# byuccl/coast

Hardware: NVIDIA B200
Metric: protected-kernel throughput (MB/s voted output), sha256 TMR (higher is better)
Workload: dtype u32

## Files before the change

### coast_b200/csrc/coast_rt.c

```c
#define _GNU_SOURCE
#include "../../include/coast_rt.h"
#include "xmr_args.h"

#include <cuda.h>
#include <ctype.h>
#include <dlfcn.h>
#include <sched.h>
#include <stdarg.h>
#include <stdio.h>
#include <stdlib.h>
#include <string.h>
#include <sys/syscall.h>
#include <unistd.h>

extern const unsigned char coast_kernels_cubin[];

__attribute__((weak)) uint32_t TMR_ERROR_CNT = 0;
__attribute__((weak)) uint64_t __SYNC_COUNT = 0;
__attribute__((weak)) void FAULT_DETECTED_DWC(void) {
    fprintf(stderr, "coast_rt: DWC mismatch detected -> FAULT_DETECTED_DWC -> abort()\n");
    abort();
}

#define DRV_FUNCS(X)                                                                                         \
// ... 469 lines not shown
    char name[64];
    snprintf(name, sizeof name, "xmr_mm_u32_%s_nc%u_inj%d", atmem ? "tct" : "tc", nc, inj);
    CUfunction fn; int occ = 1;
    int rc = get_fn(name, smem, &fn, &occ); if (rc) return rc;
    CUtensorMap ma, mb;
    {
        cuuint64_t gdim[3] = { d->K, d->M, 4 };
        cuuint64_t gstr[2] = { (cuuint64_t)d->K, (cuuint64_t)d->M * d->K };
        cuuint32_t box[3] = { 128, 128, 4 };
        cuuint32_t estr[3] = { 1, 1, 1 };
        DRV(p_cuTensorMapEncodeTiled(&ma, CU_TENSOR_MAP_DATA_TYPE_UINT8, 3, (void*)pa, gdim, gstr, box, estr,
                                     CU_TENSOR_MAP_INTERLEAVE_NONE, CU_TENSOR_MAP_SWIZZLE_128B,
                                     CU_TENSOR_MAP_L2_PROMOTION_L2_256B, CU_TENSOR_MAP_FLOAT_OOB_FILL_NONE));
    }
    {
        cuuint64_t gdim[3] = { d->K, d->N, 4 };
        cuuint64_t gstr[2] = { (cuuint64_t)d->K, (cuuint64_t)d->N * d->K };
        cuuint32_t box[3] = { 128, bn, 4 };
        cuuint32_t estr[3] = { 1, 1, 1 };
        DRV(p_cuTensorMapEncodeTiled(&mb, CU_TENSOR_MAP_DATA_TYPE_UINT8, 3, (void*)pb, gdim, gstr, box, estr,
                                     CU_TENSOR_MAP_INTERLEAVE_NONE, CU_TENSOR_MAP_SWIZZLE_128B,
                                     CU_TENSOR_MAP_L2_PROMOTION_L2_256B, CU_TENSOR_MAP_FLOAT_OOB_FILL_NONE));
    }
    unsigned tiles = (d->M / 128u) * (d->N / bn);
    unsigned grid = tiles < (unsigned)G.sm_count ? tiles : (unsigned)G.sm_count;
    void* params[3] = { a, &ma, &mb };
    if (d->flags & COAST_F_VERBOSE) fprintf(stderr, "coast_rt: %s grid=%u smem=%u tiles=%u\n", name, grid, smem, tiles);
    DRV(p_cuLaunchKernel(fn, grid, 1, 1, 256, 1, 1, smem, stream, params, NULL));
    return COAST_OK;
}
static int launch_mm_tc(const coast_launch_desc* d, xmr_args* a, int inj, CUstream stream, int atmem) {
    const size_t a_bytes = (size_t)d->M * d->K * 4u, b_bytes = (size_t)d->K * d->N * 4u;
    CUdeviceptr planes = 0;
    DRV(p_cuMemAllocFromPoolAsync(&planes, a_bytes + b_bytes, G.pool, stream));
    int rc = launch_mm_tc_planes(d, a, inj, stream, atmem, planes, planes + a_bytes);
    p_cuMemFreeAsync(planes, stream);
    return rc;
}

static int launch_impl(const coast_launch_desc* d, void* stream) {
    int rc = ensure_ctx(); if (rc) return rc;
    if (!d) return fail(COAST_ERR_BAD_ARG, "null descriptor");
    if (d->kernel >= COAST_K_COUNT_) return fail(COAST_ERR_BAD_ARG, "unknown kernel id %u", d->kernel);
    if (d->num_clones < 1 || d->num_clones > 3) return fail(COAST_ERR_BAD_ARG, "num_clones must be 1, 2 (DWC) or 3 (TMR)");
    if (d->n_units == 0) return COAST_OK;
    if (!d->d_in || !d->d_out) return fail(COAST_ERR_BAD_ARG, "null device buffer");
    const uint32_t nc = d->num_clones;
    const uint32_t upw = 32u / nc;
    const int inj = d->plan && d->plan->mode != COAST_PLAN_NONE;

    xmr_args a; memset(&a, 0, sizeof a);
    a.in = d->d_in; a.out = d->d_out; a.aux = d->d_aux;
    a.n_units = d->n_units; a.unit_base = d->unit_base;
    a.counters = (unsigned long long*)(G.peer_counters ? G.peer_counters : G.counters);
    a.status = (unsigned char*)d->d_status;
    a.unit_bytes = d->unit_bytes; a.flags = d->flags; a.mode = d->mode;
    a.M = d->M; a.N = d->N; a.K = d->K;
    memcpy(a.key, d->key, 16);
    if (inj) {
        a.plan_mode = d->plan->mode; a.seed_lo = d->plan->seed_lo; a.seed_hi = d->plan->seed_hi;
        a.threshold = d->plan->threshold; a.plan_table = (const unsigned int*)d->plan->d_table;
        if (a.plan_mode == COAST_PLAN_TABLE && !a.plan_table) return fail(COAST_ERR_BAD_ARG, "TABLE plan without d_table");
        if (a.plan_mode > COAST_PLAN_TABLE) return fail(COAST_ERR_BAD_ARG, "unknown fault plan mode %u", a.plan_mode);
    }
    a.n_sites = coast_fault_sites(d->kernel, d->unit_bytes, d->K);
    const int store_votes = store_votes_wanted(d->flags) && nc > 1;
    if (store_votes && !store_votes_built(d->kernel)) {
        static const char* const kname[COAST_K_COUNT_] = { "crc16", "sha256", "aes128", "mm_u32", "gemm_tf32", "qsort", "chstone_sha", "chstone_aes" };
        const char* strict = getenv("COAST_STRICT_FLAGS");
        if (strict && strcmp(strict, "0"))
            return fail(COAST_ERR_UNSUPPORTED, "-noMemReplication / -storeDataSync: the %s kernel has no in-loop store votes "
                                               "(COAST_STRICT_FLAGS is set)", kname[d->kernel]);
        if (!(G.warned_store_votes & (1u << d->kernel))) {
            G.warned_store_votes |= 1u << d->kernel;
            fprintf(stderr, "coast_rt: WARNING: -noMemReplication / -storeDataSync are NOT honoured by the %s kernel: it has no in-loop "
                            "store votes and runs the default sync set (SoR-exit votes only).  COAST_STRICT_FLAGS=1 makes this an error.\n",
                    kname[d->kernel]);
        }
    }
    if (store_votes && store_votes_built(d->kernel)) a.flags |= XMR_F_STORE_VOTES;

    char name[64];
    unsigned smem = 0; int tma = 0; int block = XMR_CTA_THREADS; int mm_tiled = 0; int qs_scratch = 0;
    unsigned tile_rows = 0, row_bytes = 0; CUtensorMapSwizzle swz = CU_TENSOR_MAP_SWIZZLE_NONE;
    const int aligned16 = (((uintptr_t)d->d_in) & 15u) == 0;
    switch (d->kernel) {
    case COAST_K_SHA256:
        if (d->unit_bytes == 64 && aligned16 && d->n_units < 0x7FFFFF00ull && !store_votes) {
            tma = 1; tile_rows = XMR_WARPS * upw; row_bytes = 64; swz = CU_TENSOR_MAP_SWIZZLE_64B;
            smem = ring_smem(tile_rows, row_bytes);
            snprintf(name, sizeof name, "xmr_sha256_b64_nc%u_inj%d", nc, inj);
            if (nc == 3 && !(d->flags & COAST_F_INTERLEAVE)) {
                block = 384; tile_rows = 128;
                smem = ((ring_smem(tile_rows, row_bytes) + 127u) & ~127u) + 2u * 4u * 2u * 8u * 32u * 4u;
                snprintf(name, sizeof name, "xmr_sha256_b64_seg_nc3_inj%d", inj);
            }
        } else {
            snprintf(name, sizeof name, "xmr_sha256_gen_nc%u_inj%d", nc, inj);
        }
        break;
    case COAST_K_CRC16:
        if (d->unit_bytes < 1 || d->unit_bytes > 255) return fail(COAST_ERR_BAD_ARG, "crc16 length is an unsigned char (1..255)");
        if (d->unit_bytes == 64 && aligned16 && d->n_units < 0x7FFFFF00ull && !store_votes) {
            tma = 1; block = nc == 1 ? 768 : 1024; tile_rows = (unsigned)(block / 32) * upw; row_bytes = 64;
            swz = CU_TENSOR_MAP_SWIZZLE_64B;
            smem = 0x20000u + ring_smem(tile_rows, row_bytes);
            snprintf(name, sizeof name, "xmr_crc16_b64_nc%u_inj%d", nc, inj);
        } else {
            snprintf(name, sizeof name, "xmr_crc16_gen_nc%u_inj%d", nc, inj);
        }
        break;
    case COAST_K_AES128:
        if ((d->mode & COAST_AES_KEY_PER_UNIT) && !d->d_aux) return fail(COAST_ERR_BAD_ARG, "per-unit keys need d_aux");
        if (!aligned16 || (((uintptr_t)d->d_out) & 15u)) return fail(COAST_ERR_BAD_ARG, "AES buffers must be 16-byte aligned");
        if ((d->mode & COAST_AES_KEY_PER_UNIT) && (((uintptr_t)d->d_aux) & 15u)) return fail(COAST_ERR_BAD_ARG, "AES per-unit keys must be 16-byte aligned");
        if (d->n_units >= 0x7FFFFF00ull) return fail(COAST_ERR_UNSUPPORTED, "AES: at most 2^31 - 257 blocks per launch (split the batch)");
        {
            const int dec = (d->mode & COAST_AES_DECRYPT) != 0, perkey = (d->mode & COAST_AES_KEY_PER_UNIT) != 0;
            tma = 1; block = 512; tile_rows = 16u * upw * (nc == 1 ? 2u : 4u); row_bytes = 16;
            smem = dec ? 0x38000u : 0x30000u;
            static const char* const stem[4] = { "xmr_aes128_enc", "xmr_aes128_dec", "xmr_aes128_enck", "xmr_aes128_deck" };
            snprintf(name, sizeof name, "%s_nc%u_inj%d", stem[dec + 2 * perkey], nc, inj);
        }
        break;
    case COAST_K_MM_U32:
        if (!d->d_aux || !d->M || !d->N || !d->K) return fail(COAST_ERR_BAD_ARG, "MM needs A (d_in), B (d_aux) and M,N,K");
        if (d->n_units != (uint64_t)d->M * d->N) return fail(COAST_ERR_BAD_ARG, "MM: n_units must be M*N");
        snprintf(name, sizeof name, "xmr_mm_u32_nc%u_inj%d", nc, inj);
        {
            const char* path = getenv("COAST_MM_PATH");
            const int want_tc = !path || !strcmp(path, "tc") || !strcmp(path, "tct");
            if (store_votes) break;
            if (want_tc && d->M % 128u == 0 && d->N % 64u == 0 && d->K % 128u == 0 && aligned16 &&
                !(((uintptr_t)d->d_aux) & 15u) && !(((uintptr_t)d->d_out) & 15u))
                return launch_mm_tc(d, &a, inj, (CUstream)stream, path ? !strcmp(path, "tct") : nc == 3);
            if (path && !strcmp(path, "naive")) break;
        }
        if (!store_votes && d->M % 64u == 0 && d->N % 128u == 0 && d->K % 16u == 0 && aligned16 && !(((uintptr_t)d->d_aux) & 15u) &&
            !(((uintptr_t)d->d_out) & 15u)) {
            mm_tiled = 1; block = (int)nc * 128; smem = 64u * 1024u;
            snprintf(name, sizeof name, "xmr_mm_u32_tiled_nc%u_inj%d", nc, inj);
        }
        break;
    case COAST_K_QSORT:
        if (d->unit_bytes < 4 || (d->unit_bytes & 3u) || d->unit_bytes > 4096u)
            return fail(COAST_ERR_BAD_ARG, "quicksort arrays are 1..1024 int32 (unit_bytes = 4*L, got %u)", d->unit_bytes);
        block = 128; qs_scratch = 1;
        snprintf(name, sizeof name, "xmr_qsort_nc%u_inj%d", nc, inj);
        break;
    case COAST_K_CHSTONE_SHA:
        if (d->unit_bytes < 64u || (d->unit_bytes & 63u) || d->unit_bytes >= (1u << 29))
            return fail(COAST_ERR_BAD_ARG, "CHStone sha streams are whole 64-byte blocks, 64 <= unit_bytes < 2^29 (got %u)", d->unit_bytes);
        if (!aligned16 || (((uintptr_t)d->d_out) & 3u)) return fail(COAST_ERR_BAD_ARG, "CHStone sha: d_in must be 16-byte and d_out 4-byte aligned");
        snprintf(name, sizeof name, "xmr_chsha_nc%u_inj%d", nc, inj);
        break;
    case COAST_K_CHSTONE_AES:
        if ((d->mode & COAST_AES_KEY_PER_UNIT) && !d->d_aux) return fail(COAST_ERR_BAD_ARG, "per-unit keys need d_aux");
        if (!aligned16 || (((uintptr_t)d->d_out) & 15u) || ((d->mode & COAST_AES_KEY_PER_UNIT) && (((uintptr_t)d->d_aux) & 15u)))
            return fail(COAST_ERR_BAD_ARG, "CHStone aes buffers must be 16-byte aligned");
        block = 512; smem = (d->mode & COAST_AES_DECRYPT) ? 0x38000u : 0x30000u;
        {
            static const char* const stem[2] = { "xmr_chaes_enc", "xmr_chaes_dec" };
            snprintf(name, sizeof name, "%s_nc%u_inj%d", stem[(d->mode & COAST_AES_DECRYPT) ? 1 : 0], nc, inj);
        }
        break;
    case COAST_K_GEMM_TF32:
        if (!d->d_aux || !d->M || !d->N || !d->K) return fail(COAST_ERR_BAD_ARG, "GEMM needs A (d_in), B (d_aux) and M,N,K");
        if (d->n_units != (uint64_t)d->M * d->N) return fail(COAST_ERR_BAD_ARG, "GEMM: n_units must be M*N");
        if (d->M % 128u || d->N % 128u || d->K % 32u)
            return fail(COAST_ERR_UNSUPPORTED, "GEMM_TF32 tiles are 128x128x32: M,N must be multiples of 128 and K of 32 (got %u,%u,%u)", d->M, d->N, d->K);
        if (!aligned16 || (((uintptr_t)d->d_aux) & 15u) || (((uintptr_t)d->d_out) & 15u)) return fail(COAST_ERR_BAD_ARG, "GEMM buffers must be 16-byte aligned");
        return launch_gemm_tf32(d, &a, inj, (CUstream)stream);
    default:
        return fail(COAST_ERR_UNSUPPORTED, "kernel %u is not built into this library yet", d->kernel);
    }
    if (d->kernel == COAST_K_SHA256 && (((uintptr_t)d->d_out) & 15u)) return fail(COAST_ERR_BAD_ARG, "SHA output must be 16-byte aligned");

    CUfunction fn; int occ = 1;
    rc = get_fn_b(name, smem, block, &fn, &occ); if (rc) return rc;
    unsigned grid;
    CUtensorMap map;
    void* params[2] = { &a, &map };
    if (tma) {
        uint64_t n_tiles = (d->n_units + tile_rows - 1) / tile_rows;
        a.n_tiles = (unsigned)n_tiles;
        unsigned loads = (tile_rows + 255u) / 256u;
        while (tile_rows % loads) ++loads;
        unsigned pack = 0;
        if (d->kernel == COAST_K_AES128) {
            pack = d->n_units % 16u == 0 ? 4u : d->n_units % 4u == 0 ? 2u : 0u;
            while (pack && (tile_rows / loads) % (1u << pack)) pack -= 2u;
            a.mode = (a.mode & ~XMR_AES_ROWPACK_MASK) | (pack << XMR_AES_ROWPACK_SHIFT);
        }
        rc = encode_rows_map(&map, d->d_in, row_bytes << pack, d->n_units >> pack, (tile_rows / loads) >> pack, swz); if (rc) return rc;
        uint64_t cap = (uint64_t)G.sm_count * (unsigned)occ;
        grid = (unsigned)(n_tiles < cap ? n_tiles : cap);
    } else if (mm_tiled) {
        grid = (d->M / 64u) * (d->N / 128u);
    } else {
        uint64_t warps = (d->n_units + upw - 1) / upw;
        uint64_t wpc = (uint64_t)block / 32u;
        uint64_t ctas = (warps + wpc - 1) / wpc;
        uint64_t cap = (uint64_t)G.sm_count * (unsigned)occ * (qs_scratch ? 1u : 4u);
        grid = (unsigned)(ctas < cap ? ctas : cap);
    }
    CUdeviceptr scratch = 0;
    if (qs_scratch) {
        size_t bytes = (size_t)grid * (size_t)(block / 32) * 32u * (size_t)d->unit_bytes;
        DRV(p_cuMemAllocFromPoolAsync(&scratch, bytes ? bytes : 4, G.pool, (CUstream)stream));
        a.aux = (const void*)scratch;
    }
    if (d->flags & COAST_F_VERBOSE)
        fprintf(stderr, "coast_rt: %s grid=%u block=%d smem=%u units=%llu\n", name, grid, block, smem,
                (unsigned long long)d->n_units);
    CUresult lr = p_cuLaunchKernel(fn, grid, 1, 1, (unsigned)block, 1, 1, smem, (CUstream)stream, params, NULL);
    if (scratch) p_cuMemFreeAsync(scratch, (CUstream)stream);
    if (lr != CUDA_SUCCESS) return drv_fail(lr, "cuLaunchKernel");
    return COAST_OK;
}

static int sync_impl(void* stream, coast_stats* out, int* dwc_fired) {
    int rc = ensure_ctx(); if (rc) return rc;
    if (G.peer_counters) {
        DRV(p_cuStreamSynchronize((CUstream)stream));
        if (out) { memset(out, 0, sizeof *out); out->first_fault_unit = ~0ull; }
        if (dwc_fired) *dwc_fired = 0;
        return COAST_OK;
    }
    DRV(p_cuMemcpyDtoHAsync_v2(G.h_counters, G.counters, XMR_CTR_COUNT * sizeof(uint64_t), (CUstream)stream));
    rc = stats_reset_impl(stream); if (rc) return rc;
    DRV(p_cuStreamSynchronize((CUstream)stream));
    coast_stats st;
    st.errors_corrected = G.h_counters[XMR_CTR_ERRORS];
    st.dwc_detected = G.h_counters[XMR_CTR_DWC];
    st.syncs = G.h_counters[XMR_CTR_SYNCS];
    st.injected = G.h_counters[XMR_CTR_INJECTED];
    st.first_fault_unit = G.h_counters[XMR_CTR_FIRST];
    TMR_ERROR_CNT += (uint32_t)st.errors_corrected;
    __SYNC_COUNT += st.syncs;
    if (out) *out = st;
    if (dwc_fired) *dwc_fired = st.dwc_detected != 0;
    return COAST_OK;
}
static int sync_guarded(void* stream, coast_stats* out, int call_handler) {
    ENTER();
    int fired = 0, rc = sync_impl(stream, out, &fired);
    leave();
    if (!rc && call_handler && fired) FAULT_DETECTED_DWC();
    return rc;
}
int coast_sync(void* stream, coast_stats* out) { return sync_guarded(stream, out, 1); }
int coast_sync_noabort(void* stream, coast_stats* out) { return sync_guarded(stream, out, 0); }
int coast_launch(const coast_launch_desc* d, void* stream) { ENTER(); LEAVE(launch_impl(d, stream)); }

int coast_counters_export(void* handle) {
    ENTER();
    int rc = ensure_ctx(); if (rc) LEAVE(rc);
    if (!handle) LEAVE(fail(COAST_ERR_BAD_ARG, "null handle"));
    CUipcMemHandle h;
    CUresult r = p_cuIpcGetMemHandle(&h, G.counters);
    if (r != CUDA_SUCCESS) LEAVE(drv_fail(r, "cuIpcGetMemHandle(counters)"));
    memcpy(handle, &h, sizeof h);
    LEAVE(COAST_OK);
}
int coast_counters_attach(const void* handle) {
    ENTER();
    int rc = ensure_ctx(); if (rc) LEAVE(rc);
    if (!handle) LEAVE(fail(COAST_ERR_BAD_ARG, "null handle"));
    if (G.peer_counters) LEAVE(fail(COAST_ERR_BAD_ARG, "already attached to a peer's counter block (coast_counters_detach first)"));
    CUipcMemHandle h; memcpy(&h, handle, sizeof h);
// ... 335 lines not shown
```

### coast_b200/csrc/xmr_args.h

```cpp
#ifndef XMR_ARGS_H_
#define XMR_ARGS_H_

typedef struct xmr_args {
    const void* in;
    void* out;
    const void* aux;
    unsigned long long n_units;
    unsigned long long unit_base;
    unsigned long long* counters;
    const unsigned int* plan_table;
    unsigned char* status;
    unsigned int unit_bytes;
    unsigned int flags;
    unsigned int mode;
    unsigned int M, N, K;
    unsigned int plan_mode, seed_lo, seed_hi, threshold;
    unsigned int n_sites;
    unsigned int n_tiles;
    unsigned char key[16];
} xmr_args;

#define XMR_F_STORE_VOTES 0x8000u
#define XMR_AES_ROWPACK_SHIFT 8u
#define XMR_AES_ROWPACK_MASK  (15u << XMR_AES_ROWPACK_SHIFT)

#define XMR_CTR_ERRORS   0
#define XMR_CTR_DWC      1
#define XMR_CTR_SYNCS    2
#define XMR_CTR_INJECTED 3
#define XMR_CTR_FIRST    4
#define XMR_CTR_COUNT    5

#define XMR_CTA_THREADS 256
#define XMR_WARPS       8
#define XMR_STAGES      2

#endif
```

### coast_b200/csrc/xmr_sha256.cuh

```cuda
#pragma once
#include "xmr_common.cuh"

namespace xmr {

__device__ __forceinline__ constexpr uint32_t sha_k(int i) {
    constexpr uint32_t K[64] = {
        0x428a2f98u, 0x71374491u, 0xb5c0fbcfu, 0xe9b5dba5u, 0x3956c25bu, 0x59f111f1u, 0x923f82a4u, 0xab1c5ed5u,
        0xd807aa98u, 0x12835b01u, 0x243185beu, 0x550c7dc3u, 0x72be5d74u, 0x80deb1feu, 0x9bdc06a7u, 0xc19bf174u,
        0xe49b69c1u, 0xefbe4786u, 0x0fc19dc6u, 0x240ca1ccu, 0x2de92c6fu, 0x4a7484aau, 0x5cb0a9dcu, 0x76f988dau,
        0x983e5152u, 0xa831c66du, 0xb00327c8u, 0xbf597fc7u, 0xc6e00bf3u, 0xd5a79147u, 0x06ca6351u, 0x14292967u,
        0x27b70a85u, 0x2e1b2138u, 0x4d2c6dfcu, 0x53380d13u, 0x650a7354u, 0x766a0abbu, 0x81c2c92eu, 0x92722c85u,
        0xa2bfe8a1u, 0xa81a664bu, 0xc24b8b70u, 0xc76c51a3u, 0xd192e819u, 0xd6990624u, 0xf40e3585u, 0x106aa070u,
        0x19a4c116u, 0x1e376c08u, 0x2748774cu, 0x34b0bcb5u, 0x391c0cb3u, 0x4ed8aa4au, 0x5b9cca4fu, 0x682e6ff3u,
        0x748f82eeu, 0x78a5636fu, 0x84c87814u, 0x8cc70208u, 0x90befffau, 0xa4506cebu, 0xbef9a3f7u, 0xc67178f2u};
    return K[i];
}

constexpr uint32_t SHA_SITES_PER_BLOCK = 536u;

__device__ __forceinline__ uint32_t rotr(uint32_t v, int n) { return __funnelshift_r(v, v, n); }
__device__ __forceinline__ uint32_t bswap(uint32_t v) { return __byte_perm(v, 0u, 0x0123u); }

template <bool INJECT>
__device__ __forceinline__ void sha_compress(uint32_t (&st)[8], uint32_t (&m)[16], uint32_t fs, uint32_t fmask) {
// ... 172 lines not shown
}

template <int NC, bool INJECT>
__device__ __forceinline__ void sha256_gen_body(const xmr_args& a) {
    constexpr int UPW = Lanes<NC>::kUnitsPerWarp;
    const int lane = threadIdx.x & 31;
    const int r = Lanes<NC>::replica(lane);
    const unsigned long long gwarp = ((unsigned long long)blockIdx.x * blockDim.x + threadIdx.x) >> 5;
    const unsigned long long nwarps = ((unsigned long long)gridDim.x * blockDim.x) >> 5;
    const uint32_t len = a.unit_bytes;
    const uint32_t nblk = (len + 8u) / 64u + 1u;
    const unsigned long long n_wtiles = (a.n_units + UPW - 1) / UPW;
    Tally tally(a);
    for (unsigned long long wt = gwarp; wt < n_wtiles; wt += nwarps) {
        const unsigned long long local = wt * UPW + Lanes<NC>::unit(lane);
        const bool valid = local < a.n_units;
        const unsigned long long gunit = a.unit_base + local;
        const uint8_t* msg = static_cast<const uint8_t*>(a.in) + (valid ? local : 0ull) * len;
        uint32_t fsite = 0xFFFFFFFFu, fmask = 0u;
        if (INJECT) {
            Fault f = fault_for_unit(a, NC, valid ? local : 0ull, [](uint32_t) { return 32u; });
            if (f.active && valid) {
                if (Lanes<NC>::voter(lane)) tally.injected++;
                if ((int)f.replica == r) { fmask = 1u << f.bit; fsite = f.site; }
            }
        }
        const bool sv = (a.flags & XMR_F_STORE_VOTES) != 0;
        const bool majority = a.flags & COAST_F_MAJORITY_D;
        uint32_t sv_bad = 0;
        uint32_t st[8];
        sha_init(st);
        const uintptr_t al = reinterpret_cast<uintptr_t>(a.in) | len;
        for (uint32_t blk = 0; blk < nblk; ++blk) {
            uint32_t m[16];
            if ((al & 15u) == 0 && blk * 64u + 64u <= len) {
#pragma unroll
                for (int c = 0; c < 4; ++c) {
                    const uint4 q = __ldg(reinterpret_cast<const uint4*>(msg + blk * 64u) + c);
                    m[4 * c + 0] = bswap(q.x); m[4 * c + 1] = bswap(q.y); m[4 * c + 2] = bswap(q.z); m[4 * c + 3] = bswap(q.w);
                }
            } else {
#pragma unroll
                for (int w = 0; w < 16; ++w) {
                    const uint32_t p = blk * 64u + 4u * w;
                    if ((al & 3u) == 0 && p + 4u <= len) m[w] = bswap(__ldg(reinterpret_cast<const uint32_t*>(msg + p)));
                    else m[w] = (sha_padded_byte(msg, len, p) << 24) | (sha_padded_byte(msg, len, p + 1) << 16) |
                                (sha_padded_byte(msg, len, p + 2) << 8) | sha_padded_byte(msg, len, p + 3);
                }
            }
            if (blk == nblk - 1) {
                m[14] = len >> 29;
                m[15] = len << 3;
            }
            uint32_t fs = (INJECT && fsite / SHA_SITES_PER_BLOCK == blk) ? fsite % SHA_SITES_PER_BLOCK : 0xFFFFFFFFu;
            if (!sv) {
                sha_compress<INJECT>(st, m, fs, fmask);
            } else {
                const uint32_t lo = blk * 64u, nmsg = len > lo ? (len - lo < 64u ? len - lo : 64u) : 0u;
#pragma unroll
                for (int w = 0; w < 16; ++w) {
                    const uint32_t nb = nmsg > 4u * w ? (nmsg - 4u * w < 4u ? nmsg - 4u * w : 4u) : 0u;
                    sv_bad += store_vote_bytes<NC>(m[w], nb, lane, majority);
                }
                sv_bad += sha_compress_sv<NC, INJECT>(st, m, fs, fmask, lane, majority);
            }
        }
        if (!sv) {
            sha_vote_store<NC>(st, static_cast<uint8_t*>(a.out), local, gunit, valid, lane, a.flags, tally);
        } else {
            uint32_t o[8], bad = 0;
#pragma unroll
            for (int i = 0; i < 8; ++i) { Voted v = vote_u32<NC, 1>(st[i], majority); o[i] = bswap(v.vote); bad += v.bad; }
            if (valid && Lanes<NC>::voter(lane)) {
                uint4* dst = reinterpret_cast<uint4*>(static_cast<uint8_t*>(a.out) + local * 32ull);
                dst[0] = make_uint4(o[0], o[1], o[2], o[3]);
                dst[1] = make_uint4(o[4], o[5], o[6], o[7]);
                tally.unit_exit<NC>(bad + sv_bad, len + 720u * nblk + 32u, a.flags, gunit);
            }
        }
    }
    tally.flush(a.counters);
}

constexpr int SEG_THREADS = 384, SEG_GROUPS = 4, SEG_TU = SEG_GROUPS * 32;

template <bool INJECT>
__device__ __forceinline__ void sha256_b64_seg_body(const xmr_args& a, const CUtensorMap* tmap) {
    using Ring = TileRing<SEG_TU, 64>;
    extern __shared__ __align__(1024) uint8_t smem_raw[];
    Ring ring;
    ring.init(smem_raw, tmap);
    uint32_t* exch = reinterpret_cast<uint32_t*>(smem_raw + ((Ring::SMEM_BYTES + 127u) & ~127u));
    const int tid = threadIdx.x, lane = tid & 31, warp = tid >> 5;
    const int g = warp / 3, r = warp - 3 * g;
    const int ul = g * 32 + lane;
    const uint32_t n_tiles = a.n_tiles;
    const bool majority = a.flags & COAST_F_MAJORITY_D;
    uint32_t tile = blockIdx.x;
    if (tile < n_tiles) ring.issue(0, tile);
    Tally tally(a);
    uint32_t it = 0;
    for (; tile < n_tiles; tile += gridDim.x, ++it) {
        const uint32_t next = tile + gridDim.x;
        if (next < n_tiles) ring.issue((it + 1u) & 1u, next);
        const uint8_t* base = ring.wait(it);
        uint32_t m[16];
        const uint8_t* row = base + ul * 64;
        const int sw = (ul >> 1) & 3;
#pragma unroll
        for (int c = 0; c < 4; ++c) {
            uint4 q = *reinterpret_cast<const uint4*>(row + ((c ^ sw) << 4));
            m[4 * c + 0] = bswap(q.x); m[4 * c + 1] = bswap(q.y); m[4 * c + 2] = bswap(q.z); m[4 * c + 3] = bswap(q.w);
        }
        __syncthreads();
        const unsigned long long local = (unsigned long long)tile * SEG_TU + ul;
        const bool valid = local < a.n_units;
        uint32_t fs0 = 0xFFFFFFFFu, fs1 = 0xFFFFFFFFu, fmask = 0u;
        if (INJECT) {
            Fault f = fault_for_unit(a, 3, valid ? local : 0ull, [](uint32_t) { return 32u; });
            if (f.active && valid) {
                if (r == 0) tally.injected++;
                if ((int)f.replica == r) {
                    fmask = 1u << f.bit;
                    if (f.site < SHA_SITES_PER_BLOCK) fs0 = f.site; else fs1 = f.site - SHA_SITES_PER_BLOCK;
                }
            }
        }
        uint32_t st[8];
        sha_init(st);
        sha_compress<INJECT>(st, m, fs0, fmask);
#pragma unroll
        for (int i = 0; i < 16; ++i) m[i] = 0u;
        m[0] = 0x80000000u; m[15] = 512u;
        sha_compress<INJECT>(st, m, fs1, fmask);

        uint32_t* ex = exch + ((it & 1u) * SEG_GROUPS + g) * (2 * 8 * 32);
        if (r > 0) {
#pragma unroll
            for (int i = 0; i < 8; ++i) ex[((r - 1) * 8 + i) * 32 + lane] = st[i];
        }
        if (g == 0) asm volatile("bar.sync 1, 96;" ::: "memory");
        else if (g == 1) asm volatile("bar.sync 2, 96;" ::: "memory");
        else if (g == 2) asm volatile("bar.sync 3, 96;" ::: "memory");
        else asm volatile("bar.sync 4, 96;" ::: "memory");
        if (r == 0) {
            uint32_t o[8], bad = 0;
#pragma unroll
            for (int i = 0; i < 8; ++i) {
                const uint32_t x = st[i], r1 = ex[i * 32 + lane], r2 = ex[(8 + i) * 32 + lane];
                const uint32_t e01 = __vcmpeq4(x, r1), e02 = __vcmpeq4(x, r2);
                const uint32_t v = majority ? ((x & r1) | (x & r2) | (r1 & r2)) : ((x & e01) | (r2 & ~e01));
                bad += __popc(~(e01 & e02)) >> 3;
                o[i] = bswap(v);
            }
            if (valid) {
                uint4* dst = reinterpret_cast<uint4*>(static_cast<uint8_t*>(a.out) + local * 32ull);
                dst[0] = make_uint4(o[0], o[1], o[2], o[3]);
                dst[1] = make_uint4(o[4], o[5], o[6], o[7]);
                tally.unit_exit<3>(bad, 32u, a.flags, a.unit_base + local);
            }
        }
    }
    tally.flush(a.counters);
}

}

#define XMR_SHA_B64_KERNEL(NC, INJ)                                                                      \
    extern "C" __global__ void __launch_bounds__(XMR_CTA_THREADS)                                        \
    xmr_sha256_b64_nc##NC##_inj##INJ(const __grid_constant__ xmr_args a, const __grid_constant__ CUtensorMap tmap) { \
        xmr::sha256_b64_body<NC, INJ != 0>(a, &tmap);                                                    \
    }
#define XMR_SHA_GEN_KERNEL(NC, INJ)                                                                      \
    extern "C" __global__ void __launch_bounds__(XMR_CTA_THREADS)                                        \
    xmr_sha256_gen_nc##NC##_inj##INJ(const __grid_constant__ xmr_args a) {                               \
        xmr::sha256_gen_body<NC, INJ != 0>(a);                                                           \
    }
XMR_SHA_B64_KERNEL(1, 0) XMR_SHA_B64_KERNEL(2, 0) XMR_SHA_B64_KERNEL(3, 0)
XMR_SHA_B64_KERNEL(1, 1) XMR_SHA_B64_KERNEL(2, 1) XMR_SHA_B64_KERNEL(3, 1)
XMR_SHA_GEN_KERNEL(1, 0) XMR_SHA_GEN_KERNEL(2, 0) XMR_SHA_GEN_KERNEL(3, 0)
XMR_SHA_GEN_KERNEL(1, 1) XMR_SHA_GEN_KERNEL(2, 1) XMR_SHA_GEN_KERNEL(3, 1)

#define XMR_SHA_B64_SEG_KERNEL(INJ)                                                                      \
    extern "C" __global__ void __launch_bounds__(xmr::SEG_THREADS)                                       \
    xmr_sha256_b64_seg_nc3_inj##INJ(const __grid_constant__ xmr_args a, const __grid_constant__ CUtensorMap tmap) { \
        xmr::sha256_b64_seg_body<INJ != 0>(a, &tmap);                                                    \
    }
XMR_SHA_B64_SEG_KERNEL(0) XMR_SHA_B64_SEG_KERNEL(1)
```

Measured before the change: 88180.

## Use 3-stage TMA ring with per-warp release and producer/consumer group barriers in SHA seg kernel

```diff
diff --git a/coast_b200/csrc/coast_rt.c b/coast_b200/csrc/coast_rt.c
--- a/coast_b200/csrc/coast_rt.c
+++ b/coast_b200/csrc/coast_rt.c
@@ -585,7 +585,7 @@
             snprintf(name, sizeof name, "xmr_sha256_b64_nc%u_inj%d", nc, inj);
             if (nc == 3 && !(d->flags & COAST_F_INTERLEAVE)) {
                 block = 384; tile_rows = 128;
-                smem = ((ring_smem(tile_rows, row_bytes) + 127u) & ~127u) + 2u * 4u * 2u * 8u * 32u * 4u;
+                smem = ((XMR_SHA_SEG_STAGES * tile_rows * row_bytes + 64u + 127u) & ~127u) + 4u * 2u * 8u * 32u * 4u;
                 snprintf(name, sizeof name, "xmr_sha256_b64_seg_nc3_inj%d", inj);
             }
         } else {
diff --git a/coast_b200/csrc/xmr_args.h b/coast_b200/csrc/xmr_args.h
--- a/coast_b200/csrc/xmr_args.h
+++ b/coast_b200/csrc/xmr_args.h
@@ -34,5 +34,6 @@
 #define XMR_CTA_THREADS 256
 #define XMR_WARPS       8
 #define XMR_STAGES      2
+#define XMR_SHA_SEG_STAGES 3
 
 #endif
diff --git a/coast_b200/csrc/xmr_sha256.cuh b/coast_b200/csrc/xmr_sha256.cuh
--- a/coast_b200/csrc/xmr_sha256.cuh
+++ b/coast_b200/csrc/xmr_sha256.cuh
@@ -278,28 +278,85 @@
     tally.flush(a.counters);
 }
 
-constexpr int SEG_THREADS = 384, SEG_GROUPS = 4, SEG_TU = SEG_GROUPS * 32;
+constexpr int SEG_THREADS = 384, SEG_WARPS = SEG_THREADS / 32, SEG_GROUPS = 4, SEG_TU = SEG_GROUPS * 32;
+
+struct SegRing {
+    static constexpr int STAGES = XMR_SHA_SEG_STAGES;
+    static constexpr uint32_t TILE_BYTES = (uint32_t)SEG_TU * 64u;
+    static constexpr uint32_t SMEM_BYTES = STAGES * TILE_BYTES + 64u;
+    static_assert(STAGES >= 3 && STAGES * 12 <= 64, "full[] and drained[] live in the 64 bytes after the tiles");
+    uint8_t* tiles;
+    uint64_t* full;
+    uint32_t* drained;
+    const CUtensorMap* tmap;
+    __device__ __forceinline__ void init(uint8_t* smem, const CUtensorMap* map, uint32_t first, uint32_t stride, uint32_t n_tiles) {
+        tiles = smem;
+        full = reinterpret_cast<uint64_t*>(smem + STAGES * TILE_BYTES);
+        drained = reinterpret_cast<uint32_t*>(full + STAGES);
+        tmap = map;
+        if (threadIdx.x == 0) {
+            tma_prefetch_desc(map);
+#pragma unroll
+            for (int s = 0; s < STAGES; ++s) { mbar_init(&full[s], 1); drained[s] = 0u; }
+            fence_barrier_init();
+#pragma unroll
+            for (int s = 0; s < STAGES; ++s)
+                if (first + s * stride < n_tiles) issue(s, first + s * stride);
+        }
+        __syncthreads();
+    }
+    __device__ __forceinline__ void issue(uint32_t s, uint32_t tile) {
+        mbar_arrive_expect_tx(&full[s], TILE_BYTES);
+        tma_load_2d(tiles + s * TILE_BYTES, tmap, &full[s], 0, (int)(tile * SEG_TU));
+    }
+    __device__ __forceinline__ const uint8_t* wait(uint32_t s, uint32_t phase) {
+        mbar_wait(&full[s], phase);
+        return tiles + s * TILE_BYTES;
+    }
+    __device__ __forceinline__ void release(uint32_t s, uint32_t refill, uint32_t n_tiles) {
+        __syncwarp();
+        if ((threadIdx.x & 31) == 0) {
+            uint32_t before;
+            asm volatile("atom.acq_rel.cta.shared::cta.inc.u32 %0, [%1], %2;"
+                         : "=r"(before) : "r"(smem_u32(&drained[s])), "r"((uint32_t)SEG_WARPS - 1u) : "memory");
+            if (before == SEG_WARPS - 1u && refill < n_tiles) issue(s, refill);
+        }
+    }
+};
+
+template <int BASE>
+__device__ __forceinline__ void group_bar_sync(int g) {
+    if (g == 0) asm volatile("bar.sync %0, 96;" ::"n"(BASE) : "memory");
+    else if (g == 1) asm volatile("bar.sync %0, 96;" ::"n"(BASE + 1) : "memory");
+    else if (g == 2) asm volatile("bar.sync %0, 96;" ::"n"(BASE + 2) : "memory");
+    else asm volatile("bar.sync %0, 96;" ::"n"(BASE + 3) : "memory");
+}
+template <int BASE>
+__device__ __forceinline__ void group_bar_arrive(int g) {
+    if (g == 0) asm volatile("bar.arrive %0, 96;" ::"n"(BASE) : "memory");
+    else if (g == 1) asm volatile("bar.arrive %0, 96;" ::"n"(BASE + 1) : "memory");
+    else if (g == 2) asm volatile("bar.arrive %0, 96;" ::"n"(BASE + 2) : "memory");
+    else asm volatile("bar.arrive %0, 96;" ::"n"(BASE + 3) : "memory");
+}
+constexpr int SEG_BAR_PUBLISHED = 1;
+constexpr int SEG_BAR_CONSUMED = 5;
 
 template <bool INJECT>
 __device__ __forceinline__ void sha256_b64_seg_body(const xmr_args& a, const CUtensorMap* tmap) {
-    using Ring = TileRing<SEG_TU, 64>;
     extern __shared__ __align__(1024) uint8_t smem_raw[];
-    Ring ring;
-    ring.init(smem_raw, tmap);
-    uint32_t* exch = reinterpret_cast<uint32_t*>(smem_raw + ((Ring::SMEM_BYTES + 127u) & ~127u));
+    const uint32_t n_tiles = a.n_tiles, stride = gridDim.x;
+    SegRing ring;
+    ring.init(smem_raw, tmap, blockIdx.x, stride, n_tiles);
+    uint32_t* exch = reinterpret_cast<uint32_t*>(smem_raw + ((SegRing::SMEM_BYTES + 127u) & ~127u));
     const int tid = threadIdx.x, lane = tid & 31, warp = tid >> 5;
     const int g = warp / 3, r = warp - 3 * g;
     const int ul = g * 32 + lane;
-    const uint32_t n_tiles = a.n_tiles;
     const bool majority = a.flags & COAST_F_MAJORITY_D;
-    uint32_t tile = blockIdx.x;
-    if (tile < n_tiles) ring.issue(0, tile);
+    uint32_t* ex = exch + g * (2 * 8 * 32);
     Tally tally(a);
-    uint32_t it = 0;
-    for (; tile < n_tiles; tile += gridDim.x, ++it) {
-        const uint32_t next = tile + gridDim.x;
-        if (next < n_tiles) ring.issue((it + 1u) & 1u, next);
-        const uint8_t* base = ring.wait(it);
+    uint32_t s = 0, phase = 0;
+    for (uint32_t tile = blockIdx.x; tile < n_tiles; tile += stride) {
+        const uint8_t* base = ring.wait(s, phase);
         uint32_t m[16];
         const uint8_t* row = base + ul * 64;
         const int sw = (ul >> 1) & 3;
@@ -308,7 +365,8 @@
             uint4 q = *reinterpret_cast<const uint4*>(row + ((c ^ sw) << 4));
             m[4 * c + 0] = bswap(q.x); m[4 * c + 1] = bswap(q.y); m[4 * c + 2] = bswap(q.z); m[4 * c + 3] = bswap(q.w);
         }
-        __syncthreads();
+        ring.release(s, tile + SegRing::STAGES * stride, n_tiles);
+        if (++s == SegRing::STAGES) { s = 0; phase ^= 1u; }
         const unsigned long long local = (unsigned long long)tile * SEG_TU + ul;
         const bool valid = local < a.n_units;
         uint32_t fs0 = 0xFFFFFFFFu, fs1 = 0xFFFFFFFFu, fmask = 0u;
@@ -330,24 +388,34 @@
         m[0] = 0x80000000u; m[15] = 512u;
         sha_compress<INJECT>(st, m, fs1, fmask);
 
-        uint32_t* ex = exch + ((it & 1u) * SEG_GROUPS + g) * (2 * 8 * 32);
         if (r > 0) {
+            if (tile != blockIdx.x) group_bar_sync<SEG_BAR_CONSUMED>(g);
 #pragma unroll
             for (int i = 0; i < 8; ++i) ex[((r - 1) * 8 + i) * 32 + lane] = st[i];
-        }
-        if (g == 0) asm volatile("bar.sync 1, 96;" ::: "memory");
-        else if (g == 1) asm volatile("bar.sync 2, 96;" ::: "memory");
-        else if (g == 2) asm volatile("bar.sync 3, 96;" ::: "memory");
-        else asm volatile("bar.sync 4, 96;" ::: "memory");
-        if (r == 0) {
+            group_bar_arrive<SEG_BAR_PUBLISHED>(g);
+        } else {
+            group_bar_sync<SEG_BAR_PUBLISHED>(g);
+            uint32_t r1[8], r2[8], diff = 0;
+#pragma unroll
+            for (int i = 0; i < 8; ++i) {
+                r1[i] = ex[i * 32 + lane];
+                r2[i] = ex[(8 + i) * 32 + lane];
+                diff |= (st[i] ^ r1[i]) | (st[i] ^ r2[i]);
+            }
+            if (tile + stride < n_tiles) group_bar_arrive<SEG_BAR_CONSUMED>(g);
             uint32_t o[8], bad = 0;
-#pragma unroll
-            for (int i = 0; i < 8; ++i) {
-                const uint32_t x = st[i], r1 = ex[i * 32 + lane], r2 = ex[(8 + i) * 32 + lane];
-                const uint32_t e01 = __vcmpeq4(x, r1), e02 = __vcmpeq4(x, r2);
-                const uint32_t v = majority ? ((x & r1) | (x & r2) | (r1 & r2)) : ((x & e01) | (r2 & ~e01));
-                bad += __popc(~(e01 & e02)) >> 3;
-                o[i] = bswap(v);
+            if (__any_sync(0xFFFFFFFFu, diff != 0u)) {
+#pragma unroll
+                for (int i = 0; i < 8; ++i) {
+                    const uint32_t x = st[i];
+                    const uint32_t e01 = __vcmpeq4(x, r1[i]), e02 = __vcmpeq4(x, r2[i]);
+                    const uint32_t v = majority ? ((x & r1[i]) | (x & r2[i]) | (r1[i] & r2[i])) : ((x & e01) | (r2[i] & ~e01));
+                    bad += __popc(~(e01 & e02)) >> 3;
+                    o[i] = bswap(v);
+                }
+            } else {
+#pragma unroll
+                for (int i = 0; i < 8; ++i) o[i] = bswap(st[i]);
             }
             if (valid) {
                 uint4* dst = reinterpret_cast<uint4*>(static_cast<uint8_t*>(a.out) + local * 32ull);
```

New measurement: 89290, median of 6. 1.3% higher.

## Decouple SHA256 TMR segment groups with per-group mbarrier TMA pipelines

Applied to the files above, without the earlier changes.

```diff
diff --git a/coast_b200/csrc/coast_rt.c b/coast_b200/csrc/coast_rt.c
--- a/coast_b200/csrc/coast_rt.c
+++ b/coast_b200/csrc/coast_rt.c
@@ -575,7 +575,7 @@
 
     char name[64];
     unsigned smem = 0; int tma = 0; int block = XMR_CTA_THREADS; int mm_tiled = 0; int qs_scratch = 0;
-    unsigned tile_rows = 0, row_bytes = 0; CUtensorMapSwizzle swz = CU_TENSOR_MAP_SWIZZLE_NONE;
+    unsigned tile_rows = 0, row_bytes = 0, box_rows = 0; CUtensorMapSwizzle swz = CU_TENSOR_MAP_SWIZZLE_NONE;
     const int aligned16 = (((uintptr_t)d->d_in) & 15u) == 0;
     switch (d->kernel) {
     case COAST_K_SHA256:
@@ -584,8 +584,8 @@
             smem = ring_smem(tile_rows, row_bytes);
             snprintf(name, sizeof name, "xmr_sha256_b64_nc%u_inj%d", nc, inj);
             if (nc == 3 && !(d->flags & COAST_F_INTERLEAVE)) {
-                block = 384; tile_rows = 128;
-                smem = ((ring_smem(tile_rows, row_bytes) + 127u) & ~127u) + 2u * 4u * 2u * 8u * 32u * 4u;
+                block = 384; tile_rows = 128; box_rows = XMR_SHA_SEG_BOX_ROWS;
+                smem = XMR_SHA_SEG_SMEM;
                 snprintf(name, sizeof name, "xmr_sha256_b64_seg_nc3_inj%d", inj);
             }
         } else {
@@ -679,6 +679,7 @@
         a.n_tiles = (unsigned)n_tiles;
         unsigned loads = (tile_rows + 255u) / 256u;
         while (tile_rows % loads) ++loads;
+        if (box_rows) loads = tile_rows / box_rows;
         unsigned pack = 0;
         if (d->kernel == COAST_K_AES128) {
             pack = d->n_units % 16u == 0 ? 4u : d->n_units % 4u == 0 ? 2u : 0u;
diff --git a/coast_b200/csrc/xmr_args.h b/coast_b200/csrc/xmr_args.h
--- a/coast_b200/csrc/xmr_args.h
+++ b/coast_b200/csrc/xmr_args.h
@@ -35,4 +35,7 @@
 #define XMR_WARPS       8
 #define XMR_STAGES      2
 
+#define XMR_SHA_SEG_BOX_ROWS 32u
+#define XMR_SHA_SEG_SMEM     49536u
+
 #endif
diff --git a/coast_b200/csrc/xmr_sha256.cuh b/coast_b200/csrc/xmr_sha256.cuh
--- a/coast_b200/csrc/xmr_sha256.cuh
+++ b/coast_b200/csrc/xmr_sha256.cuh
@@ -279,38 +279,106 @@
 }
 
 constexpr int SEG_THREADS = 384, SEG_GROUPS = 4, SEG_TU = SEG_GROUPS * 32;
+constexpr int SEG_ROWS = XMR_SHA_SEG_BOX_ROWS, SEG_STAGES = 4, SEG_AHEAD = 2, SEG_SLOTS = 2;
+constexpr uint32_t SEG_STAGE_BYTES = SEG_ROWS * 64u;
+constexpr uint32_t SEG_SLOT_BYTES = 2u * 8u * 32u * 4u;
+constexpr uint32_t SEG_EXCH_OFF = SEG_GROUPS * SEG_STAGES * SEG_STAGE_BYTES;
+constexpr uint32_t SEG_BAR_OFF = SEG_EXCH_OFF + SEG_GROUPS * SEG_SLOTS * SEG_SLOT_BYTES;
+constexpr int SEG_BARS_PER_GROUP = 2 * SEG_STAGES + 2 * SEG_SLOTS;
+static_assert(SEG_BAR_OFF + SEG_GROUPS * SEG_BARS_PER_GROUP * 8u == XMR_SHA_SEG_SMEM, "host and kernel disagree on the shared-memory size");
+static_assert(SEG_AHEAD < SEG_STAGES, "a stage is refilled only after it was released");
+
+__device__ __forceinline__ void seg_wait(uint32_t bar, uint32_t parity) {
+    asm volatile(
+        "{\n\t.reg .pred p;\n\t"
+        "WAIT_%=:\n\t"
+        "mbarrier.try_wait.parity.shared::cta.b64 p, [%0], %1;\n\t"
+        "@p bra DONE_%=;\n\t"
+        "bra WAIT_%=;\n\t"
+        "DONE_%=:\n\t}" ::"r"(bar), "r"(parity) : "memory");
+}
+__device__ __forceinline__ void seg_arrive(uint32_t bar) {
+    asm volatile("mbarrier.arrive.shared::cta.b64 _, [%0];" ::"r"(bar) : "memory");
+}
+__device__ __forceinline__ uint32_t seg_keep(uint32_t v) { asm volatile("mov.b32 %0, %0;" : "+r"(v)); return v; }
+__device__ __forceinline__ uint4 seg_lds128(uint32_t addr) {
+    uint4 v;
+    asm volatile("ld.shared.v4.u32 {%0, %1, %2, %3}, [%4];" : "=r"(v.x), "=r"(v.y), "=r"(v.z), "=r"(v.w) : "r"(addr) : "memory");
+    return v;
+}
+__device__ __forceinline__ void seg_sts128(uint32_t addr, uint32_t x, uint32_t y, uint32_t z, uint32_t w) {
+    asm volatile("st.shared.v4.u32 [%0], {%1, %2, %3, %4};" ::"r"(addr), "r"(x), "r"(y), "r"(z), "r"(w) : "memory");
+}
 
 template <bool INJECT>
 __device__ __forceinline__ void sha256_b64_seg_body(const xmr_args& a, const CUtensorMap* tmap) {
-    using Ring = TileRing<SEG_TU, 64>;
     extern __shared__ __align__(1024) uint8_t smem_raw[];
-    Ring ring;
-    ring.init(smem_raw, tmap);
-    uint32_t* exch = reinterpret_cast<uint32_t*>(smem_raw + ((Ring::SMEM_BYTES + 127u) & ~127u));
     const int tid = threadIdx.x, lane = tid & 31, warp = tid >> 5;
     const int g = warp / 3, r = warp - 3 * g;
-    const int ul = g * 32 + lane;
-    const uint32_t n_tiles = a.n_tiles;
+    const uint32_t sm = smem_u32(smem_raw);
+    const uint32_t tiles = sm + g * (SEG_STAGES * SEG_STAGE_BYTES);
+    const uint32_t exch = sm + SEG_EXCH_OFF + g * (SEG_SLOTS * SEG_SLOT_BYTES);
+    const uint32_t full = sm + SEG_BAR_OFF + g * (SEG_BARS_PER_GROUP * 8);
+    constexpr uint32_t EMPTY = SEG_STAGES * 8, XFULL = 2 * SEG_STAGES * 8, XEMPTY = XFULL + SEG_SLOTS * 8;
+    if (tid == 0) {
+        tma_prefetch_desc(tmap);
+        uint64_t* const bars = reinterpret_cast<uint64_t*>(smem_raw + SEG_BAR_OFF);
+        for (int k = 0; k < SEG_GROUPS; ++k) {
+            uint64_t* const b = bars + k * SEG_BARS_PER_GROUP;
+#pragma unroll
+            for (int s = 0; s < SEG_STAGES; ++s) { mbar_init(&b[s], 1); mbar_init(&b[SEG_STAGES + s], 3); }
+#pragma unroll
+            for (int s = 0; s < SEG_SLOTS; ++s) { mbar_init(&b[2 * SEG_STAGES + s], 64); mbar_init(&b[2 * SEG_STAGES + SEG_SLOTS + s], 32); }
+        }
+        fence_barrier_init();
+    }
+    __syncthreads();
+
+    const uint32_t n_q = (uint32_t)((a.n_units + SEG_ROWS - 1) / SEG_ROWS);
+    const uint32_t n_units = (uint32_t)a.n_units;
+    const uint32_t stride = seg_keep(gridDim.x * SEG_GROUPS);
+    const bool producer = r == 1 && lane == 0;
+    auto issue = [&](uint32_t i, uint32_t q) {
+        const uint32_t s = i % SEG_STAGES;
+        asm volatile("mbarrier.arrive.expect_tx.shared::cta.b64 _, [%0], %1;" ::"r"(full + 8 * s), "r"(SEG_STAGE_BYTES) : "memory");
+        asm volatile("cp.async.bulk.tensor.2d.shared::cluster.global.tile.mbarrier::complete_tx::bytes [%0], [%1, {%3, %4}], [%2];"
+                     ::"r"(tiles + s * SEG_STAGE_BYTES), "l"(tmap), "r"(full + 8 * s), "r"(0), "r"((int)(q * SEG_ROWS)) : "memory");
+    };
+    uint32_t q = blockIdx.x * SEG_GROUPS + g;
+    if (producer) {
+#pragma unroll
+        for (uint32_t i = 0; i < (uint32_t)SEG_AHEAD; ++i)
+            if (q + i * stride < n_q) issue(i, q + i * stride);
+    }
+    const uint32_t row = seg_keep(tiles + lane * 64 + ((((uint32_t)lane >> 1) & 3u) << 4));
+    const uint32_t ex_lane = seg_keep(exch + lane * 16);
     const bool majority = a.flags & COAST_F_MAJORITY_D;
-    uint32_t tile = blockIdx.x;
-    if (tile < n_tiles) ring.issue(0, tile);
     Tally tally(a);
-    uint32_t it = 0;
-    for (; tile < n_tiles; tile += gridDim.x, ++it) {
-        const uint32_t next = tile + gridDim.x;
-        if (next < n_tiles) ring.issue((it + 1u) & 1u, next);
-        const uint8_t* base = ring.wait(it);
+    uint32_t exits = 0;
+    for (uint32_t it = 0; q < n_q; q += stride, ++it) {
+        const uint32_t s = it % SEG_STAGES;
+        seg_wait(full + 8 * s, (it / SEG_STAGES) & 1u);
         uint32_t m[16];
-        const uint8_t* row = base + ul * 64;
-        const int sw = (ul >> 1) & 3;
+        const uint32_t ra = row + s * SEG_STAGE_BYTES;
 #pragma unroll
         for (int c = 0; c < 4; ++c) {
-            uint4 q = *reinterpret_cast<const uint4*>(row + ((c ^ sw) << 4));
-            m[4 * c + 0] = bswap(q.x); m[4 * c + 1] = bswap(q.y); m[4 * c + 2] = bswap(q.z); m[4 * c + 3] = bswap(q.w);
-        }
-        __syncthreads();
-        const unsigned long long local = (unsigned long long)tile * SEG_TU + ul;
-        const bool valid = local < a.n_units;
+            const uint4 v = seg_lds128(ra ^ (c << 4));
+            m[4 * c + 0] = bswap(v.x); m[4 * c + 1] = bswap(v.y); m[4 * c + 2] = bswap(v.z); m[4 * c + 3] = bswap(v.w);
+        }
+        __syncwarp();
+        if (lane == 0) seg_arrive(full + EMPTY + 8 * s);
+        if (producer) {
+            const uint32_t ahead = q + SEG_AHEAD * stride;
+            if (ahead < n_q) {
+                if (it >= (uint32_t)(SEG_STAGES - SEG_AHEAD)) {
+                    const uint32_t old = it + SEG_AHEAD - SEG_STAGES;
+                    seg_wait(full + EMPTY + 8 * (old % SEG_STAGES), (old / SEG_STAGES) & 1u);
+                }
+                issue(it + SEG_AHEAD, ahead);
+            }
+        }
+        const uint32_t local = q * SEG_ROWS + lane;
+        const bool valid = local < n_units;
         uint32_t fs0 = 0xFFFFFFFFu, fs1 = 0xFFFFFFFFu, fmask = 0u;
         if (INJECT) {
             Fault f = fault_for_unit(a, 3, valid ? local : 0ull, [](uint32_t) { return 32u; });
@@ -330,33 +398,50 @@
         m[0] = 0x80000000u; m[15] = 512u;
         sha_compress<INJECT>(st, m, fs1, fmask);
 
-        uint32_t* ex = exch + ((it & 1u) * SEG_GROUPS + g) * (2 * 8 * 32);
+        const uint32_t slot = it % SEG_SLOTS, use = it / SEG_SLOTS;
+        const uint32_t ex = ex_lane + slot * SEG_SLOT_BYTES;
         if (r > 0) {
-#pragma unroll
-            for (int i = 0; i < 8; ++i) ex[((r - 1) * 8 + i) * 32 + lane] = st[i];
-        }
-        if (g == 0) asm volatile("bar.sync 1, 96;" ::: "memory");
-        else if (g == 1) asm volatile("bar.sync 2, 96;" ::: "memory");
-        else if (g == 2) asm volatile("bar.sync 3, 96;" ::: "memory");
-        else asm volatile("bar.sync 4, 96;" ::: "memory");
-        if (r == 0) {
-            uint32_t o[8], bad = 0;
-#pragma unroll
-            for (int i = 0; i < 8; ++i) {
-                const uint32_t x = st[i], r1 = ex[i * 32 + lane], r2 = ex[(8 + i) * 32 + lane];
-                const uint32_t e01 = __vcmpeq4(x, r1), e02 = __vcmpeq4(x, r2);
-                const uint32_t v = majority ? ((x & r1) | (x & r2) | (r1 & r2)) : ((x & e01) | (r2 & ~e01));
-                bad += __popc(~(e01 & e02)) >> 3;
-                o[i] = bswap(v);
+            if (use > 0) seg_wait(full + XEMPTY + 8 * slot, (use - 1u) & 1u);
+            seg_sts128(ex + (2 * (r - 1) + 0) * 512, st[0], st[1], st[2], st[3]);
+            seg_sts128(ex + (2 * (r - 1) + 1) * 512, st[4], st[5], st[6], st[7]);
+            seg_arrive(full + XFULL + 8 * slot);
+        } else {
+            seg_wait(full + XFULL + 8 * slot, use & 1u);
+            const uint4 a0 = seg_lds128(ex), a1 = seg_lds128(ex + 512), b0 = seg_lds128(ex + 1024), b1 = seg_lds128(ex + 1536);
+            seg_arrive(full + XEMPTY + 8 * slot);
+            const uint32_t r1[8] = {a0.x, a0.y, a0.z, a0.w, a1.x, a1.y, a1.z, a1.w};
+            const uint32_t r2[8] = {b0.x, b0.y, b0.z, b0.w, b1.x, b1.y, b1.z, b1.w};
+            uint32_t o[8], bad = 0, d = 0;
+#pragma unroll
+            for (int i = 0; i < 8; ++i) d |= (st[i] ^ r1[i]) | (st[i] ^ r2[i]);
+            if (seg_keep(d) == 0) {
+#pragma unroll
+                for (int i = 0; i < 8; ++i) o[i] = bswap(st[i]);
+            } else {
+#pragma unroll
+                for (int i = 0; i < 8; ++i) {
+                    const uint32_t x = st[i];
+                    const uint32_t e01 = __vcmpeq4(x, r1[i]), e02 = __vcmpeq4(x, r2[i]);
+                    const uint32_t v = majority ? ((x & r1[i]) | (x & r2[i]) | (r1[i] & r2[i])) : ((x & e01) | (r2[i] & ~e01));
+                    bad += __popc(~(e01 & e02)) >> 3;
+                    o[i] = bswap(v);
+                }
             }
             if (valid) {
-                uint4* dst = reinterpret_cast<uint4*>(static_cast<uint8_t*>(a.out) + local * 32ull);
+                uint4* dst = reinterpret_cast<uint4*>(static_cast<uint8_t*>(a.out) + (unsigned long long)local * 32ull);
                 dst[0] = make_uint4(o[0], o[1], o[2], o[3]);
                 dst[1] = make_uint4(o[4], o[5], o[6], o[7]);
-                tally.unit_exit<3>(bad, 32u, a.flags, a.unit_base + local);
-            }
-        }
-    }
+                ++exits;
+                if (bad) {
+                    if (a.flags & COAST_F_COUNT_ERRORS_D) tally.errors += bad;
+                    const unsigned long long gunit = a.unit_base + local;
+                    if (gunit < tally.first) tally.first = gunit;
+                }
+                if (tally.status) tally.status[local] = (unsigned char)(bad > 255u ? 255u : bad);
+            }
+        }
+    }
+    if ((a.flags & COAST_F_COUNT_ERRORS_D) && (a.flags & COAST_F_COUNT_SYNCS_D)) tally.syncs += 32u * exits;
     tally.flush(a.counters);
 }
 
```

Measured after the change: 88100 before, 89190 after (median of 6 runs). 1.01x the previous value.
